# david-wb/tiny-diffusion

Hardware: AMD Instinct MI355X
Metric: train images/s (q_sample+fwd+MSE+bwd+allreduce+Adam), MNIST 28x28 UNet fp32; 1000-step sample latency in `sample` (higher is better)
Workload: dtype f32; 1 GPU; diffusion.py unconditional MNIST 28x28 UNet, fp32, train step, batch 256/GPU (BASELINE.json configs[1]); global_batch=256, per_gpu_batch=256, parallelism=dp1

## Files before the change

include/tdx.h:

```cpp
#ifndef TDX_H
#define TDX_H

#include <stddef.h>
#include <stdint.h>

#ifdef __cplusplus
extern "C" {
#endif

#define TDX_VERSION 400

#define TDX_E_BADARG (-1)
#define TDX_E_SHAPE (-2)
#define TDX_E_WORKSPACE (-3)
#define TDX_E_STATE (-4)

typedef void* tdx_stream_t;

int tdx_version(void);
const char* tdx_error_string(int code);


int tdx_q_sample(const float* x0, const float* noise, const int64_t* t,
                 const float* sqrt_ac, const float* sqrt_1mac, float* x_t,
// ... 65 lines not shown
int tdx_final_conv_backward(const float* in, const float* g_out, const float* w, float* g_in, float* dw, float* db,
                            float* scratch, int B, int H, int W, int cout, tdx_stream_t stream);

int tdx_conv3x3_fwd(const float* in, const float* wpk, const float* bias, float* out,
                    int B, int H, int W, int cin, int cout, int flags,
                    const float* in_scale, const float* in_shift,
                    const float* out_scale, const float* out_shift,
                    float* stats_partial, tdx_stream_t stream);
int tdx_conv3x3_fwd_splitk(const float* in, const float* wpk, const float* bias, float* out,
                           int B, int H, int W, int cin, int cout, int flags,
                           const float* in_scale, const float* in_shift,
                           const float* out_scale, const float* out_shift,
                           float* scratch, size_t scratch_floats, tdx_stream_t stream);
size_t tdx_conv3x3_splitk_scratch_floats(int B, int H, int W, int cin, int cout);
int tdx_conv3x3_wino_ok(int B, int H, int W, int cin, int cout);
int tdx_pack_conv3x3_wino(const float* w_oihw, float* u_fwd, float* u_dgrad, int cout, int cin, tdx_stream_t stream);
int tdx_conv3x3_fwd_wino(const float* in, const float* u, const float* bias, float* out, int B, int H, int W,
                         int cin, int cout, int flags, const float* out_scale, const float* out_shift,
                         float* stats_partial, tdx_stream_t stream);
int tdx_conv3x3_fwd_wino_infer(const float* in, const float* u, const float* bias, float* out, int B, int H, int W,
                               int cin, int cout, const float* out_scale, const float* out_shift, float* scratch,
                               size_t scratch_floats, tdx_stream_t stream);
int tdx_conv3x3_train_algo(int B, int H, int W, int cin, int cout, int role);
int tdx_conv3x3_infer_algo(int B, int H, int W, int cin, int cout);
int tdx_conv3x3_wgrad_wino_splits(int B, int H, int W, int cin, int cout);
int tdx_conv3x3_wgrad_wino(const float* in, const float* dy, float* dw_slabs, int B, int H, int W, int cin, int cout,
                           tdx_stream_t stream);
int tdx_conv3x3_wino_stat_tiles(int B, int H, int W);
int tdx_conv3x3_wino_stat_tile_rows(int B, int H, int W);
int tdx_pack_conv3x3_tiled(const float* w_oihw, float* w_tiled, int cout, int cin, tdx_stream_t stream);
int tdx_conv3x3_fwd_infer(const float* in, const float* w_tiled, const float* bias, float* out, int B, int H, int W,
                          int cin, int cout, const float* out_scale, const float* out_shift, float* scratch,
                          size_t scratch_floats, tdx_stream_t stream);
size_t tdx_conv3x3_infer_scratch_floats(int B, int H, int W, int cin, int cout);
int tdx_conv3x3_fwd_train(const float* in, const float* wpk, const float* bias, float* out, int B, int H, int W,
                          int cin, int cout, int flags, float* stats_partial, float* scratch,
                          size_t scratch_floats, tdx_stream_t stream);
size_t tdx_conv3x3_train_scratch_floats(int B, int H, int W, int cin, int cout);
int tdx_conv3x3_stat_tiles(int B, int H, int W, int cin, int cout);
int tdx_conv3x3_stat_tile_rows(int B, int H, int W, int cin, int cout);
int tdx_conv3x3_shape_ok(int B, int H, int W, int cin, int cout);
int tdx_conv3x3_tile_shape(int B, int H, int W, int cin, int cout, int role);

int tdx_conv3x3_dgrad(const float* dy, const float* w_dgrad, float* dx, int B, int H, int W,
                      int cin, int cout, tdx_stream_t stream);

// ... 184 lines not shown
```

tiny_diffusion_amd/_lib.py:

```python
from __future__ import annotations

import ctypes as C
import os

import torch

from . import _build

_c_float_p = C.c_void_p
_c_i64_p = C.c_void_p
_ptr = C.c_void_p


class TdxError(RuntimeError):
    pass


def _load():
    path = _build.LIB
    if not os.path.exists(path):
        if os.environ.get("TDX_NO_AUTOBUILD"):
            raise TdxError(
                f"{path} not found: build it with `python -m tiny_diffusion_amd._build` "
                "(there is no CPU fallback for the HIP path)"
# ... 29 lines not shown
    "tdx_mse_loss": (C.c_int, [_ptr, _ptr, _ptr, _ptr, C.c_float, C.c_int64, _ptr]),
    "tdx_mse_scratch_bytes": (C.c_size_t, []),
    "tdx_mse_loss_grad": (C.c_int, [_ptr, _ptr, _ptr, _ptr, C.c_float, C.c_int64, _ptr, _ptr]),
    "tdx_adam_step": (C.c_int, [_ptr, _ptr, _ptr, _ptr, C.c_int64, C.c_float, C.c_float, C.c_float,
                                C.c_float, C.c_int, C.c_float, _ptr]),
    "tdx_adam_clip_scratch_bytes": (C.c_size_t, []),
    "tdx_adam_step_clip": (C.c_int, [_ptr, _ptr, _ptr, _ptr, C.c_int64, C.c_float, C.c_float, C.c_float, C.c_float,
                                     C.c_int, C.c_float, C.c_float, _ptr, _ptr, _ptr]),
    "tdx_edge_conv_wgrad_scratch_floats": (C.c_size_t, [C.c_int] * 3),
    "tdx_initial_conv_forward": (C.c_int, [_ptr, _ptr, _ptr, _ptr, C.c_int, C.c_int, C.c_int, C.c_int, C.c_int, _ptr]),
    "tdx_initial_conv_backward": (C.c_int, [_ptr, _ptr, _ptr, _ptr, _ptr, C.c_int, C.c_int, C.c_int, C.c_int, C.c_int,
                                            _ptr]),
    "tdx_final_conv_forward": (C.c_int, [_ptr, _ptr, _ptr, _ptr, C.c_int, C.c_int, C.c_int, C.c_int, _ptr]),
    "tdx_final_conv_backward": (C.c_int, [_ptr, _ptr, _ptr, _ptr, _ptr, _ptr, _ptr, C.c_int, C.c_int, C.c_int, C.c_int,
                                          _ptr]),
    "tdx_pack_conv3x3": (C.c_int, [_ptr, _ptr, _ptr, C.c_int, C.c_int, _ptr]),
    "tdx_conv3x3_wino_ok": (C.c_int, [C.c_int] * 5),
    "tdx_pack_conv3x3_wino": (C.c_int, [_ptr, _ptr, _ptr, C.c_int, C.c_int, _ptr]),
    "tdx_conv3x3_fwd_wino": (C.c_int, [_ptr, _ptr, _ptr, _ptr, C.c_int, C.c_int, C.c_int, C.c_int, C.c_int, C.c_int, _ptr,
                                       _ptr, _ptr, _ptr]),
    "tdx_conv3x3_fwd_wino_infer": (C.c_int, [_ptr, _ptr, _ptr, _ptr, C.c_int, C.c_int, C.c_int, C.c_int, C.c_int, _ptr, _ptr,
                                             _ptr, C.c_size_t, _ptr]),
    "tdx_conv3x3_train_algo": (C.c_int, [C.c_int] * 6),
    "tdx_conv3x3_infer_algo": (C.c_int, [C.c_int] * 5),
    "tdx_conv3x3_wgrad_wino_splits": (C.c_int, [C.c_int] * 5),
    "tdx_conv3x3_wgrad_wino": (C.c_int, [_ptr, _ptr, _ptr, C.c_int, C.c_int, C.c_int, C.c_int, C.c_int, _ptr]),
    "tdx_conv3x3_wino_stat_tiles": (C.c_int, [C.c_int] * 3),
    "tdx_conv3x3_wino_stat_tile_rows": (C.c_int, [C.c_int] * 3),
    "tdx_pack_conv3x3_tiled": (C.c_int, [_ptr, _ptr, C.c_int, C.c_int, _ptr]),
    "tdx_conv3x3_fwd_infer": (C.c_int, [_ptr, _ptr, _ptr, _ptr, C.c_int, C.c_int, C.c_int, C.c_int, C.c_int, _ptr, _ptr,
                                        _ptr, C.c_size_t, _ptr]),
    "tdx_conv3x3_infer_scratch_floats": (C.c_size_t, [C.c_int] * 5),
    "tdx_conv3x3_fwd": (C.c_int, [_ptr, _ptr, _ptr, _ptr, C.c_int, C.c_int, C.c_int, C.c_int, C.c_int,
                                  C.c_int, _ptr, _ptr, _ptr, _ptr, _ptr, _ptr]),
    "tdx_conv3x3_fwd_splitk": (C.c_int, [_ptr, _ptr, _ptr, _ptr, C.c_int, C.c_int, C.c_int, C.c_int, C.c_int,
                                         C.c_int, _ptr, _ptr, _ptr, _ptr, _ptr, C.c_size_t, _ptr]),
    "tdx_conv3x3_splitk_scratch_floats": (C.c_size_t, [C.c_int] * 5),
    "tdx_conv3x3_fwd_train": (C.c_int, [_ptr, _ptr, _ptr, _ptr, C.c_int, C.c_int, C.c_int, C.c_int, C.c_int, C.c_int,
                                        _ptr, _ptr, C.c_size_t, _ptr]),
    "tdx_conv3x3_train_scratch_floats": (C.c_size_t, [C.c_int] * 5),
    "tdx_conv3x3_stat_tiles": (C.c_int, [C.c_int] * 5),
    "tdx_conv3x3_stat_tile_rows": (C.c_int, [C.c_int] * 5),
    "tdx_conv3x3_wgrad_splits": (C.c_int, [C.c_int] * 5),
    "tdx_diag_conv_occupancy": (C.c_int, [C.c_int]),
    "tdx_conv3x3_wgrad_splits_bf16": (C.c_int, [C.c_int] * 5),
    "tdx_conv3x3_fwd_bf16_io": (C.c_int, [_ptr] * 4 + [C.c_int] * 6 + [_ptr] * 5 + [C.c_int, _ptr]),
# ... 133 lines not shown
```

tiny_diffusion_amd/csrc/conv3x3.hip:

```cpp
#include "internal.h"
#include <cstring>
#include <type_traits>

#define BK 32
#define BKP 36

#include "conv_shared.h"

template <int BM, int BN, bool IN_BN, int EPI>
__global__ void __launch_bounds__(256)
conv3x3_igemm_kernel(ConvArgs a) {
  constexpr int WGM = 2, WGN = 2;
  constexpr int WTM = BM / WGM, WTN = BN / WGN;
  constexpr int TM = WTM / 32, TN = WTN / 32;
  constexpr int AI = BM / 32, BI = BN / 32;
  static_assert(TM >= 1 && TN >= 1, "wave tile must hold a 32x32 MFMA tile");

  extern __shared__ __attribute__((aligned(16))) float smem[];
  float* As = smem;
  float* Bs = smem + 2 * BM * BKP;

  const int tid = threadIdx.x;
  const int lane = tid & 63, wave = tid >> 6;
  const int l31 = lane & 31, half = lane >> 5;
// ... 776 lines not shown
  if (!strcmp(key, "time_proj_early")) { g_tdx_time_proj_early = value != 0; return 0; }
  if (!strcmp(key, "time_stage_diag")) { g_tdx_time_stage = value == 6 ? 6 : 14; return 0; }
  if (!strcmp(key, "time_l1_impl")) { g_tdx_time_l1_impl = value; return 0; }
  if (!strcmp(key, "input_copy")) { g_tdx_input_copy = value; return 0; }
  if (!strcmp(key, "conv_dbg")) { g_conv_dbg = value; return 0; }
  if (!strcmp(key, "bf16_materialize")) { g_tdx_bf16_materialize = value ? 1 : 0; return 0; }
  if (!strcmp(key, "bf16_thin")) { g_tdx_bf16_thin = value < 0 ? 0 : value; return 0; }
  if (!strcmp(key, "bf16_ring")) { g_tdx_bf16_ring = value ? 1 : 0; return 0; }
  if (!strcmp(key, "bf16_wgrad9")) { g_tdx_wgrad9 = value ? 1 : 0; return 0; }
  if (!strcmp(key, "bf16_wgrad_swz")) { g_tdx_wgrad_bf16s = value ? 1 : 0; return 0; }
  if (!strcmp(key, "conv_stamp")) { g_conv_stamp = value; g_tdx_probe_stamp = value; return 0; }
  if (!strcmp(key, "wgrad_small")) { g_wgrad_small = value; return 0; }
  if (!strcmp(key, "wino")) { g_tdx_wino = value != 0; return 0; }
  if (!strcmp(key, "wino_infer")) { g_tdx_wino_infer = value != 0; return 0; }
  if (!strcmp(key, "wino_infer_min_units")) { g_tdx_wino_infer_min_units = value >= 0 ? value : 700; return 0; }
  if (!strcmp(key, "wino_infer_ovh")) { g_wino_infer_ovh = value >= 0 ? value : 2; return 0; }
  if (!strcmp(key, "wino_infer_red")) { g_wino_infer_red = value >= 0 ? value : 3; return 0; }
  if (!strcmp(key, "wino_wgrad")) { g_tdx_wino_wgrad = value != 0; return 0; }
  if (!strcmp(key, "wino_wgrad_min_tiles")) { g_tdx_wino_wgrad_min_tiles = value > 0 ? value : 1024; return 0; }
  if (!strcmp(key, "wino_wgrad_target")) { g_tdx_wino_wgrad_target = value > 0 ? value : 512; return 0; }
  if (!strcmp(key, "wino_min_wgs")) { g_tdx_wino_min_wgs = value > 0 ? value : 1; return 0; }
  if (!strcmp(key, "wino_rows")) { g_tdx_wino_rows = value != 0; return 0; }
  if (!strcmp(key, "wino_rows_min_stages")) { g_tdx_wino_rows_min_stages = value > 0 ? value : 16; return 0; }
  if (!strcmp(key, "infer_ring")) { g_tdx_infer_ring = value != 0; return 0; }
  if (!strcmp(key, "infer_stages")) { g_infer_stages = value == 3 ? 3 : 4; return 0; }
  if (!strcmp(key, "infer_splits")) { g_infer_splits = value > 0 ? value : 0; return 0; }
  if (!strcmp(key, "infer_ovh")) { g_infer_ovh = value >= 0 ? value : 4; return 0; }
  if (!strcmp(key, "infer_red")) { g_infer_red = value >= 0 ? value : 12; return 0; }
  if (!strcmp(key, "infer_cus")) { g_tdx_infer_cus = value > 0 && value <= 256 ? value : 256; return 0; }
  if (!strcmp(key, "wgrad9_wgs")) { g_wgrad9_wgs = value > 0 ? value : 0; return 0; }
  if (!strcmp(key, "wgrad_plan")) { g_wgrad_plan = value; return 0; }
  if (!strcmp(key, "wgrad_rounds")) { g_wgrad_rounds = value; return 0; }
  if (!strcmp(key, "conv_dma")) { g_conv_dma = value; return 0; }
  if (!strcmp(key, "wgrad_target")) { g_wgrad_target = value > 0 ? value : 2048; return 0; }
  if (!strcmp(key, "wgrad_target_big")) { g_wgrad_target_big = value > 0 ? value : 0; return 0; }
  return TDX_E_BADARG;
}

static TileCfg pick_tile(int64_t M, int cout) {
  const TileCfg cands[3] = {{128, 128}, {128, 64}, {64, 64}};
  if (g_force_tile >= 1 && g_force_tile <= 3 && cout % cands[g_force_tile - 1].bn == 0)
    return cands[g_force_tile - 1];
  for (int i = 0; i < 3; ++i) {
    if (cout % cands[i].bn) continue;
    if (i == 2) return cands[i];
    const int64_t tiles = ((M + cands[i].bm - 1) / cands[i].bm) * (cout / cands[i].bn);
// ... 1187 lines not shown
```

tiny_diffusion_amd/csrc/conv3x3_wino.hip:

```cpp
#include "internal.h"
#include "conv_shared.h"

extern unsigned* g_tdx_diag_buffer;
extern size_t g_tdx_diag_bytes;
extern int g_tdx_probe_stamp;

constexpr int WT = 64;
constexpr int WN = 64;
constexpr int WK = 8;
constexpr int A_ST = 16 * WT * WK;
constexpr int B_ST = 16 * WN * WK;
constexpr int STAGE = A_ST + B_ST;

struct WinoArgs {
  const float* in;
  const float* u;
  const float* bias;
  float* out;
  const float* out_scale;
  const float* out_shift;
  float* stats;
  int B, H, W, Cin, Cout, th, tw, NT, tilesN, M;
  float rcp_tpi, rcp_tw;
  int per;
  int compact;
  unsigned long long* stamps;
};

constexpr int OLD = 68;
constexpr int TAB_OFF = 2 * STAGE;
typedef unsigned u32x4 __attribute__((ext_vector_type(4)));

template <int EPI, int XH = -1>
__device__ __forceinline__ void wino_epilogue(const WinoArgs& a, float* out, const float* bias, f32x16 (&acc)[16], float* smem,
                                              int tblk, int n0, int wm, int wn, int l31, int half, int tid,
                                              const f32x4* xin = nullptr) {
#if defined(__HIP_DEVICE_COMPILE__)
  const unsigned* tab = reinterpret_cast<const unsigned*>(smem + TAB_OFF);
  const int cl = wn * 32 + l31, col = n0 + cl;
  const float bv = bias ? bias[col] : 0.f;
  float osc = 1.f, osh = 0.f;
  if (EPI == EPI_BNRELU) { osc = a.out_scale[col]; osh = a.out_shift[col]; }
  float csum = 0.f, cnt = 0.f;
  float* ot = smem;
  f32x4 pv[8];
#pragma unroll
  for (int r = 0; r < 16; ++r) {
    if (XH >= 0 && (r & 3) == 0) {
#pragma unroll
      for (int p = 0; p < 8; ++p) pv[p] = xin[(p * 4 + (r >> 2)) * 64];
    }
    auto M = [&](int p) { return XH >= 0 && (p >> 3) != XH ? pv[p & 7][r & 3] : acc[p][r]; };
    float s0[4], s1[4];
#pragma unroll
    for (int nu = 0; nu < 4; ++nu) {
      s0[nu] = M(0 + nu) + M(4 + nu) + M(8 + nu);
      s1[nu] = M(4 + nu) - M(8 + nu) - M(12 + nu);
    }
    float y[4] = {s0[0] + s0[1] + s0[2], s0[1] - s0[2] - s0[3], s1[0] + s1[1] + s1[2], s1[1] - s1[2] - s1[3]};
    const int tl = wm * 32 + (r & 3) + 8 * (r >> 2) + 4 * half;
    const unsigned m = tab[2 * tl + 1];
#pragma unroll
    for (int q = 0; q < 4; ++q) {
      float val = y[q] + bv;
      if (EPI == EPI_BNRELU) val = fmaxf(fmaf(val, osc, osh), 0.f);
      const bool ok = (m >> q) & 1u;
      if (XH < 0) ot[(tl * 4 + q) * OLD + cl] = val;
      csum += ok ? val : 0.f;
      cnt += ok ? 1.f : 0.f;
      y[q] = ok ? val : 0.f;
    }
    acc[0][r] = y[0]; acc[1][r] = y[1]; acc[4][r] = y[2]; acc[5][r] = y[3];
    acc[2][r] = (m & 1u) ? 1.f : 0.f;
    acc[3][r] = (m & 2u) ? 1.f : 0.f;
    acc[6][r] = (m & 4u) ? 1.f : 0.f;
    acc[7][r] = (m & 8u) ? 1.f : 0.f;
  }
  if (XH >= 0) {
    __syncthreads();
#pragma unroll
    for (int r = 0; r < 16; ++r) {
      const int tl = wm * 32 + (r & 3) + 8 * (r >> 2) + 4 * half;
      ot[(tl * 4 + 0) * OLD + cl] = acc[0][r]; ot[(tl * 4 + 1) * OLD + cl] = acc[1][r];
      ot[(tl * 4 + 2) * OLD + cl] = acc[4][r]; ot[(tl * 4 + 3) * OLD + cl] = acc[5][r];
    }
  }
  __syncthreads();
  {
    const auto rsrc_out = __builtin_amdgcn_make_buffer_rsrc(out, 0, (int)((int64_t)a.M * a.Cout * 4), 0x00020000);
    const int c4 = (tid & 15) * 4, q = (tid >> 4) & 3;
    const unsigned qoff = (unsigned)((((q >> 1) * a.W + (q & 1)) * a.Cout + n0 + c4) * 4);
    const uint2* tab2 = reinterpret_cast<const uint2*>(tab);
    const float* src = ot + (tid >> 4) * OLD + c4;
#pragma unroll
    for (int i = 0; i < 16; ++i) {
      const uint2 e = tab2[4 * i + (tid >> 6)];
      const unsigned off = ((e.y >> q) & 1u) ? e.x + qoff : 0x80000000u;
      const f32x4 v = *reinterpret_cast<const f32x4*>(src + i * 16 * OLD);
      __builtin_amdgcn_raw_buffer_store_b128(__builtin_bit_cast(u32x4, v), rsrc_out, off, 0, 0);
    }
  }
  if (EPI == EPI_STATS) {
    float* red = smem + 256 * OLD;
    const float s = csum + __shfl_xor(csum, 32, 64);
    const float n = cnt + __shfl_xor(cnt, 32, 64);
    if (half == 0) { red[wm * 64 + cl] = s; red[128 + wm * 64 + cl] = n; }
    __syncthreads();
    if (tid < 64) {
      const float ts = red[tid] + red[64 + tid];
      const float tn = red[128 + tid] + red[192 + tid];
      red[256 + tid] = tn > 0.f ? ts / tn : 0.f;
      a.stats[((size_t)tblk * 2 + 0) * a.Cout + n0 + tid] = ts;
    }
    __syncthreads();
    const float mean = red[256 + cl];
    float q = 0.f;
#pragma unroll
    for (int r = 0; r < 16; ++r) {
      const float d0 = acc[0][r] - mean, d1 = acc[1][r] - mean, d2 = acc[4][r] - mean, d3 = acc[5][r] - mean;
      q = fmaf(d0 * acc[2][r], d0, q); q = fmaf(d1 * acc[3][r], d1, q);
      q = fmaf(d2 * acc[6][r], d2, q); q = fmaf(d3 * acc[7][r], d3, q);
    }
    q += __shfl_xor(q, 32, 64);
    __syncthreads();
    if (half == 0) red[wm * 64 + cl] = q;
    __syncthreads();
    if (tid < 64) a.stats[((size_t)tblk * 2 + 1) * a.Cout + n0 + tid] = red[tid] + red[64 + tid];
  }
#endif
}

#if defined(__HIP_DEVICE_COMPILE__)
__device__ __forceinline__ float s_add(float x, float y) { float r; asm("v_add_f32 %0, %1, %2" : "=v"(r) : "v"(x), "v"(y)); return r; }
__device__ __forceinline__ float s_sub(float x, float y) { float r; asm("v_sub_f32 %0, %1, %2" : "=v"(r) : "v"(x), "v"(y)); return r; }
__device__ __forceinline__ f32x4 add4(f32x4 x, f32x4 y) { return f32x4{s_add(x[0], y[0]), s_add(x[1], y[1]), s_add(x[2], y[2]), s_add(x[3], y[3])}; }
__device__ __forceinline__ f32x4 sub4(f32x4 x, f32x4 y) { return f32x4{s_sub(x[0], y[0]), s_sub(x[1], y[1]), s_sub(x[2], y[2]), s_sub(x[3], y[3])}; }
#endif

__device__ __forceinline__ int div_rcp(int n, int d, float r, int* rem) {
  int q = (int)((float)n * r);
  int m = n - q * d;
  if (m < 0) { --q; m += d; }
  else if (m >= d) { ++q; m -= d; }
  *rem = m;
  return q;
}

template <int EPI, bool SPLITK, bool ROWS>
__global__ void __launch_bounds__(256)
conv3x3_wino_kernel(WinoArgs a) {
// ... 274 lines not shown
        }
      };
      if (PEEL) stage(std::true_type{}, 0);
      for (int s = PEEL ? 1 : 0; s < ns; ++s) stage(std::false_type{}, s);
      asm volatile("s_waitcnt vmcnt(0) lgkmcnt(0)\n\ts_barrier" ::: "memory");
    }
    if (a.stamps) { t_loop = __builtin_amdgcn_s_memrealtime(); c_loop = __builtin_amdgcn_s_memtime() - c_loop; }
    if (SPLITK)
      wino_epilogue<EPI_PLAIN>(a, a.out + (size_t)blockIdx.y * (size_t)a.M * a.Cout, nullptr, acc, smem, tblk, n0, wm, wn, l31, half, tid);
    else
      wino_epilogue<EPI>(a, a.out, a.bias, acc, smem, tblk, n0, wm, wn, l31, half, tid);
  }
  if (a.stamps && tid == 0) {
    asm volatile("s_waitcnt vmcnt(0)" ::: "memory");
    unsigned long long* o = a.stamps + 8 * ((size_t)blockIdx.y * gridDim.x + blockIdx.x);
    o[0] = t_entry; o[1] = t_issued; o[2] = t_landed; o[3] = t_loop; o[4] = __builtin_amdgcn_s_memrealtime();
    o[5] = c_loop;
    o[6] = __builtin_amdgcn_s_getreg(4 | (0 << 6) | (31 << 11));
    o[7] = __builtin_amdgcn_s_getreg(20 | (0 << 6) | (3 << 11)) & 0xf;
  }
#endif
}

__global__ void __launch_bounds__(512) pack_wino_batch_kernel(TdxWinoPackBatch b) {
  int u = 0;
  while (u + 1 < b.count && (int)blockIdx.x >= b.start[u + 1]) ++u;
  const int cin = b.cin[u], cout = b.cout[u], cin_real = b.cin_real[u];
  const int blk = blockIdx.x - b.start[u];
  const int nkb = cin / 8;
  const int cb = blk / nkb, kb = blk - cb * nkb;
  const int cl = threadIdx.x >> 3, k8 = threadIdx.x & 7;
  const int co = cb * 64 + cl, ci = kb * 8 + k8;
  float g[9];
#pragma unroll
  for (int tap = 0; tap < 9; ++tap) g[tap] = ci < cin_real ? b.w[u][((size_t)co * cin_real + ci) * 9 + tap] : 0.f;
  float gg[4][3], U[16];
#pragma unroll
  for (int c = 0; c < 3; ++c) {
    gg[0][c] = g[c];
    gg[1][c] = 0.5f * (g[c] + g[3 + c] + g[6 + c]);
    gg[2][c] = 0.5f * (g[c] - g[3 + c] + g[6 + c]);
    gg[3][c] = g[6 + c];
  }
#pragma unroll
  for (int r = 0; r < 4; ++r) {
    U[r * 4 + 0] = gg[r][0];
// ... 53 lines not shown
  pack_wino_batch_kernel<<<blocks, 512, 0, to_stream(stream)>>>(*b);
  TDX_CHECK_LAUNCH();
  return 0;
}

int tdx_pack_conv3x3_wino_pad(const float* w_oihw, float* u_fwd, float* u_dgrad, int cout, int cin_real, int cin,
                              tdx_stream_t stream) {
  if (!w_oihw || cout <= 0 || cin <= 0 || cin_real <= 0 || cin_real > cin) return TDX_E_BADARG;
  if (cin % 64 || cout % 64) return TDX_E_SHAPE;
  if (!u_fwd && !u_dgrad) return 0;
  TdxWinoPackBatch b{};
  b.count = 1;
  b.w[0] = w_oihw; b.uf[0] = u_fwd; b.ud[0] = u_dgrad; b.cout[0] = cout; b.cin[0] = cin; b.cin_real[0] = cin_real;
  return tdx_pack_conv3x3_wino_batch(&b, stream);
}

extern "C" int tdx_pack_conv3x3_wino(const float* w_oihw, float* u_fwd, float* u_dgrad, int cout, int cin,
                                     tdx_stream_t stream) {
  return tdx_pack_conv3x3_wino_pad(w_oihw, u_fwd, u_dgrad, cout, cin, cin, stream);
}

int g_tdx_wino_rows = 1;
int g_tdx_wino_rows_min_stages = 16;

int tdx_conv3x3_wino_launch(const float* in, const float* u, const float* bias, float* out, int B, int H, int W,
                            int cin, int cout, int flags, const float* out_scale, const float* out_shift,
                            float* stats_partial, int splits, int per, tdx_stream_t stream) {
  if (!in || !u || !out) return TDX_E_BADARG;
  if (!tdx_conv3x3_wino_ok(B, H, W, cin, cout)) return TDX_E_SHAPE;
  if (flags & ~(TDX_CONV_OUT_BNRELU | TDX_CONV_OUT_STATS)) return TDX_E_BADARG;
  if ((flags & TDX_CONV_OUT_BNRELU) && (!out_scale || !out_shift)) return TDX_E_BADARG;
  if ((flags & TDX_CONV_OUT_STATS) && (!stats_partial || (flags & TDX_CONV_OUT_BNRELU))) return TDX_E_BADARG;
  if (splits < 1 || (splits > 1 && (per < 1 || (int64_t)per * (splits - 1) >= cin / WK))) return TDX_E_BADARG;
  WinoArgs a{};
  a.in = in; a.u = u; a.bias = bias; a.out = out; a.out_scale = out_scale; a.out_shift = out_shift;
  a.stats = stats_partial;
  a.B = B; a.H = H; a.W = W; a.Cin = cin; a.Cout = cout;
  a.th = (H + 1) / 2; a.tw = (W + 1) / 2;
  a.NT = B * a.th * a.tw;
  a.rcp_tpi = 1.0f / (float)(a.th * a.tw); a.rcp_tw = 1.0f / (float)a.tw;
  a.tilesN = cout / WN;
  a.M = B * H * W;
  a.per = per;
  a.compact = cdiv(a.NT, WT) < 64;
  const dim3 grid(a.compact ? cdiv(a.NT, WT) * a.tilesN : (cdiv(a.NT, WT) + 7) / 8 * 8 * a.tilesN, splits);
  a.stamps = g_tdx_probe_stamp == 3 && g_tdx_diag_buffer && (size_t)grid.x * grid.y * 64 <= g_tdx_diag_bytes
                 ? reinterpret_cast<unsigned long long*>(g_tdx_diag_buffer) : nullptr;
  const size_t lds = (size_t)2 * STAGE * sizeof(float) + WT * 2 * sizeof(unsigned);
  hipStream_t st = to_stream(stream);
#define TDX_WINO_LAUNCH(EPI_, SPL_, ROWS_)                                                                       \
  do {                                                                                                           \
    auto kern = conv3x3_wino_kernel<EPI_, SPL_, ROWS_>;                                                          \
    static bool attr_set = false;                                                                                \
    if (!attr_set) {                                                                                             \
      hipError_t e = hipFuncSetAttribute(reinterpret_cast<const void*>(kern),                                    \
                                         hipFuncAttributeMaxDynamicSharedMemorySize, (int)lds);                  \
      if (e != hipSuccess) return (int)e;                                                                        \
      attr_set = true;                                                                                           \
    }                                                                                                            \
    kern<<<grid, 256, lds, st>>>(a);                                                                             \
  } while (0)
  const bool rows = g_tdx_wino_rows && cin / WK >= g_tdx_wino_rows_min_stages;
  if (splits > 1) TDX_WINO_LAUNCH(EPI_PLAIN, true, false);
  else if (flags & TDX_CONV_OUT_BNRELU) TDX_WINO_LAUNCH(EPI_BNRELU, false, false);
  else if (flags & TDX_CONV_OUT_STATS) {
    if (rows) TDX_WINO_LAUNCH(EPI_STATS, false, true);
    else TDX_WINO_LAUNCH(EPI_STATS, false, false);
  } else if (rows) TDX_WINO_LAUNCH(EPI_PLAIN, false, true);
  else TDX_WINO_LAUNCH(EPI_PLAIN, false, false);
#undef TDX_WINO_LAUNCH
  TDX_CHECK_LAUNCH();
  return 0;
}

extern "C" int tdx_conv3x3_fwd_wino(const float* in, const float* u, const float* bias, float* out, int B, int H, int W,
                                    int cin, int cout, int flags, const float* out_scale, const float* out_shift,
                                    float* stats_partial, tdx_stream_t stream) {
  return tdx_conv3x3_wino_launch(in, u, bias, out, B, H, W, cin, cout, flags, out_scale, out_shift, stats_partial, 1, 0,
                                 stream);
}

constexpr int GT8 = 8;
constexpr int XS_F = GT8 * 16 * 64;
constexpr int ES_F = GT8 * 4 * 64;
constexpr int WST_F = XS_F + ES_F;
constexpr int WNST = 3;
constexpr int WG_MAX_CHUNK = 1024;
constexpr int WG_XCH_F = 4 * 8 * 16 * 64;
constexpr size_t WG_LDS = 131072;
static_assert((size_t)WNST * WST_F * 4 + (size_t)WG_MAX_CHUNK * 4 <= WG_LDS && (size_t)WG_XCH_F * 4 <= WG_LDS, "LDS");

struct WinoWgArgs {
  const float* in;
// ... 330 lines not shown
```

tiny_diffusion_amd/csrc/internal.h:

```cpp
#pragma once
#include "common.h"

int tdx_copy_floats(const float* src, float* dst, size_t n, hipStream_t st);
int tdx_copy_segments(const float* const* src, float* const* dst, const size_t* n, int count, hipStream_t st);
int tdx_pixel_sum(const void* g, float* out, int B, int HW, int C, hipStream_t st, int io16 = 0);
int tdx_reduce_partials(const float* partial, float* out, int nblk, int stride, int count,
                        hipStream_t st);
int tdx_initial_conv_fwd(const float* x, const float* w, const float* bias, void* out, int B, int H,
                         int W, int cin, int cout_real, hipStream_t st, int io16 = 0);
int tdx_small_conv_wgrad_blocks(int B, int H, int W);
int tdx_small_conv_partial_width(void);
int tdx_initial_conv_wgrad(const float* x, const void* g, float* partial, float* dw, float* db,
                           int B, int H, int W, int cin, int cout_real, hipStream_t st, int io16 = 0);
int tdx_initial_conv_dgrad(const void* g_x0, const float* w, float* g_x, int B, int H, int W, int cin,
                           int cout_real, hipStream_t st, int io16 = 0);
int tdx_final_conv_fwd(const void* in, const float* w, const float* bias, float* out, int B, int H,
                       int W, int cout, hipStream_t st, int io16 = 0);
int tdx_final_conv_fwd_psample(const void* in, const float* w, const float* bias, float* eps_out, int B, int H, int W,
                               int cout, float* x, const float* z, const float* coef, const int32_t* t_idx,
                               uint64_t seed, int philox, int64_t* counter_dec, hipStream_t st, int io16 = 0,
                               int64_t elem0 = 0, const int64_t* tau = nullptr);
int tdx_final_conv_dgrad(const float* g_out, const float* w, void* g_in, int B, int H, int W,
                         int cout, hipStream_t st, int io16 = 0);
int tdx_final_conv_wgrad(const void* in, const float* g_out, float* partial, float* dw, float* db,
// ... 23 lines not shown
#define TDX_PACK_MAX 13
struct TdxPackBatch {
  const float* w[TDX_PACK_MAX];
  float* wf[TDX_PACK_MAX];
  float* wd[TDX_PACK_MAX];
  int cout[TDX_PACK_MAX], cin[TDX_PACK_MAX], cin_real[TDX_PACK_MAX], chunk_start[TDX_PACK_MAX];
  int count;
};
int tdx_pack_conv3x3_batch(TdxPackBatch* b, tdx_stream_t stream);
struct TdxWinoPackBatch {
  const float* w[TDX_PACK_MAX];
  float* uf[TDX_PACK_MAX];
  float* ud[TDX_PACK_MAX];
  int cout[TDX_PACK_MAX], cin[TDX_PACK_MAX], cin_real[TDX_PACK_MAX], start[TDX_PACK_MAX];
  int count;
};
int tdx_pack_conv3x3_wino_batch(TdxWinoPackBatch* b, tdx_stream_t stream);
extern "C" int tdx_conv3x3_wino_ok(int B, int H, int W, int cin, int cout);
extern "C" int tdx_conv3x3_wino_stat_tiles(int B, int H, int W);
extern "C" int tdx_conv3x3_wino_stat_tile_rows(int B, int H, int W);
extern int g_tdx_wino, g_tdx_wino_min_wgs;
extern int g_tdx_wino_wgrad, g_tdx_wino_wgrad_min_tiles, g_tdx_wino_wgrad_target;
extern int g_tdx_wino_rows, g_tdx_wino_rows_min_stages;
extern "C" int tdx_conv3x3_wgrad_wino_splits(int B, int H, int W, int cin, int cout);
extern "C" int tdx_conv3x3_wgrad_wino(const float* in, const float* dy, float* dw_slabs, int B, int H, int W, int cin, int cout,
                                      tdx_stream_t stream);
extern int g_tdx_wino_infer_min_units;
extern int g_tdx_wino_infer;
int tdx_conv3x3_wino_launch(const float* in, const float* u, const float* bias, float* out, int B, int H, int W,
                            int cin, int cout, int flags, const float* out_scale, const float* out_shift,
                            float* stats_partial, int splits, int per, tdx_stream_t stream);
int tdx_conv3x3_fwd_wino_infer_ex(const float* in, const float* u, const float* bias, float* out, int B, int H, int W,
                                  int cin, int cout, const float* out_scale, const float* out_shift, float* scratch,
                                  size_t scratch_floats, tdx_stream_t stream, TdxSplitDefer* defer, TdxPoolFuse* pool);
int tdx_pack_conv3x3_tiled_batch(TdxPackBatch* b, tdx_stream_t stream);
int tdx_pack_conv3x3_tiled_pad(const float* w_oihw, float* w_tiled, int cout, int cin_real, int cin, tdx_stream_t stream);
int tdx_pack_conv3x3_batch_bf16(TdxPackBatch* b, tdx_stream_t stream);
int tdx_pack_conv3x3_pad(const float* w_oihw, float* w_fwd, float* w_dgrad, int cout, int cin_real,
                         int cin, tdx_stream_t stream);
int tdx_conv3x3_wgrad_reduce_pad(const float* dw_slabs, float* dw_oihw, int splits, int cout, int cin,
                                 int cin_real, tdx_stream_t stream);
int tdx_time_embed_bwd_ex(const float* tf, const int64_t* y, const float* const* P, float* const* G,
                          const float* pre, const float* emb, const float* const* gk, const int* ldg,
                          const int* widths, float* scratch, int B, int ncls, hipStream_t st,
                          const int64_t* t_i64 = nullptr, int td = 0, int parts = 7);
int tdx_bn_moments(const float* stats_partial, int tiles, int tile_rows, int64_t count, int C, double* mom,
// ... 77 lines not shown
```

Measured before the change: 27090 images/s.

## Split Winograd conv tail wave into half-width workgroups to balance CUs

```diff
diff --git a/include/tdx.h b/include/tdx.h
--- a/include/tdx.h
+++ b/include/tdx.h
@@ -111,6 +111,9 @@
                                int cin, int cout, const float* out_scale, const float* out_shift, float* scratch,
                                size_t scratch_floats, tdx_stream_t stream);
 int tdx_conv3x3_train_algo(int B, int H, int W, int cin, int cout, int role);
+int tdx_conv3x3_wino_tail_plan(int B, int H, int W, int cout, int cus, int* plan);
+int tdx_conv3x3_wino_tail_wg(int B, int H, int W, int cout, int cus, int id, int* wg);
+int tdx_conv3x3_wino_tail_last(int* plan);
 int tdx_conv3x3_infer_algo(int B, int H, int W, int cin, int cout);
 int tdx_conv3x3_wgrad_wino_splits(int B, int H, int W, int cin, int cout);
 int tdx_conv3x3_wgrad_wino(const float* in, const float* dy, float* dw_slabs, int B, int H, int W, int cin, int cout,
diff --git a/tiny_diffusion_amd/_lib.py b/tiny_diffusion_amd/_lib.py
--- a/tiny_diffusion_amd/_lib.py
+++ b/tiny_diffusion_amd/_lib.py
@@ -75,6 +75,9 @@
     "tdx_conv3x3_fwd_wino_infer": (C.c_int, [_ptr, _ptr, _ptr, _ptr, C.c_int, C.c_int, C.c_int, C.c_int, C.c_int, _ptr, _ptr,
                                              _ptr, C.c_size_t, _ptr]),
     "tdx_conv3x3_train_algo": (C.c_int, [C.c_int] * 6),
+    "tdx_conv3x3_wino_tail_plan": (C.c_int, [C.c_int] * 5 + [C.POINTER(C.c_int)]),
+    "tdx_conv3x3_wino_tail_wg": (C.c_int, [C.c_int] * 6 + [C.POINTER(C.c_int)]),
+    "tdx_conv3x3_wino_tail_last": (C.c_int, [C.POINTER(C.c_int)]),
     "tdx_conv3x3_infer_algo": (C.c_int, [C.c_int] * 5),
     "tdx_conv3x3_wgrad_wino_splits": (C.c_int, [C.c_int] * 5),
     "tdx_conv3x3_wgrad_wino": (C.c_int, [_ptr, _ptr, _ptr, C.c_int, C.c_int, C.c_int, C.c_int, C.c_int, _ptr]),
diff --git a/tiny_diffusion_amd/csrc/conv3x3.hip b/tiny_diffusion_amd/csrc/conv3x3.hip
--- a/tiny_diffusion_amd/csrc/conv3x3.hip
+++ b/tiny_diffusion_amd/csrc/conv3x3.hip
@@ -822,6 +822,8 @@
   if (!strcmp(key, "wino_min_wgs")) { g_tdx_wino_min_wgs = value > 0 ? value : 1; return 0; }
   if (!strcmp(key, "wino_rows")) { g_tdx_wino_rows = value != 0; return 0; }
   if (!strcmp(key, "wino_rows_min_stages")) { g_tdx_wino_rows_min_stages = value > 0 ? value : 16; return 0; }
+  if (!strcmp(key, "wino_tail_max_rounds")) { g_tdx_wino_tail_max_rounds = value >= 0 ? value : 3; return 0; }
+  if (!strcmp(key, "wino_tail")) { g_tdx_wino_tail = value & 3; return 0; }
   if (!strcmp(key, "infer_ring")) { g_tdx_infer_ring = value != 0; return 0; }
   if (!strcmp(key, "infer_stages")) { g_infer_stages = value == 3 ? 3 : 4; return 0; }
   if (!strcmp(key, "infer_splits")) { g_infer_splits = value > 0 ? value : 0; return 0; }
diff --git a/tiny_diffusion_amd/csrc/conv3x3_wino.hip b/tiny_diffusion_amd/csrc/conv3x3_wino.hip
--- a/tiny_diffusion_amd/csrc/conv3x3_wino.hip
+++ b/tiny_diffusion_amd/csrc/conv3x3_wino.hip
@@ -1,3 +1,4 @@
+#include <mutex>
 #include "internal.h"
 #include "conv_shared.h"
 
@@ -25,17 +26,40 @@
   int per;
   int compact;
   unsigned long long* stamps;
+  int nb;
+  int half_f0;
 };
+
+__host__ __device__ inline void wino_real_wg(int f, int nb, int tilesN, int compact, int* tblk, int* nblk) {
+  if (compact) { *tblk = f / tilesN; *nblk = f - *tblk * tilesN; return; }
+  const int g8 = 8 * tilesN, nfull = (nb >> 3) * g8;
+  if (f < nfull) {
+    const int xb = f / g8, xr = f - xb * g8;
+    *tblk = xb * 8 + (xr & 7); *nblk = xr >> 3;
+  } else {
+    const int rem = nb & 7, fr = f - nfull;
+    *nblk = fr / rem; *tblk = (nb & ~7) + (fr - *nblk * rem);
+  }
+}
+static int wino_real_id(int f, int nb, int tilesN, int compact) {
+  if (compact) return f;
+  int tblk, nblk;
+  wino_real_wg(f, nb, tilesN, compact, &tblk, &nblk);
+  return (tblk >> 3) * 8 * tilesN + nblk * 8 + (tblk & 7);
+}
 
 constexpr int OLD = 68;
 constexpr int TAB_OFF = 2 * STAGE;
 typedef unsigned u32x4 __attribute__((ext_vector_type(4)));
 
-template <int EPI, int XH = -1>
+template <int EPI, int XH = -1, bool HALF = false>
 __device__ __forceinline__ void wino_epilogue(const WinoArgs& a, float* out, const float* bias, f32x16 (&acc)[16], float* smem,
                                               int tblk, int n0, int wm, int wn, int l31, int half, int tid,
                                               const f32x4* xin = nullptr) {
 #if defined(__HIP_DEVICE_COMPILE__)
+  static_assert(!HALF || XH >= 0, "the half-width workgroup runs the row split");
+  constexpr bool ACTIVE = !HALF || XH == 0;
+  constexpr int NW = HALF ? 32 : 64;
   const unsigned* tab = reinterpret_cast<const unsigned*>(smem + TAB_OFF);
   const int cl = wn * 32 + l31, col = n0 + cl;
   const float bv = bias ? bias[col] : 0.f;
@@ -45,7 +69,7 @@
   float* ot = smem;
   f32x4 pv[8];
 #pragma unroll
-  for (int r = 0; r < 16; ++r) {
+  for (int r = 0; r < (ACTIVE ? 16 : 0); ++r) {
     if (XH >= 0 && (r & 3) == 0) {
 #pragma unroll
       for (int p = 0; p < 8; ++p) pv[p] = xin[(p * 4 + (r >> 2)) * 64];
@@ -79,7 +103,7 @@
   if (XH >= 0) {
     __syncthreads();
 #pragma unroll
-    for (int r = 0; r < 16; ++r) {
+    for (int r = 0; r < (ACTIVE ? 16 : 0); ++r) {
       const int tl = wm * 32 + (r & 3) + 8 * (r >> 2) + 4 * half;
       ot[(tl * 4 + 0) * OLD + cl] = acc[0][r]; ot[(tl * 4 + 1) * OLD + cl] = acc[1][r];
       ot[(tl * 4 + 2) * OLD + cl] = acc[4][r]; ot[(tl * 4 + 3) * OLD + cl] = acc[5][r];
@@ -88,15 +112,16 @@
   __syncthreads();
   {
     const auto rsrc_out = __builtin_amdgcn_make_buffer_rsrc(out, 0, (int)((int64_t)a.M * a.Cout * 4), 0x00020000);
-    const int c4 = (tid & 15) * 4, q = (tid >> 4) & 3;
+    constexpr int LP = NW / 4, RI = 256 / LP;
+    const int c4 = (tid & (LP - 1)) * 4, q = (tid / LP) & 3;
     const unsigned qoff = (unsigned)((((q >> 1) * a.W + (q & 1)) * a.Cout + n0 + c4) * 4);
     const uint2* tab2 = reinterpret_cast<const uint2*>(tab);
-    const float* src = ot + (tid >> 4) * OLD + c4;
-#pragma unroll
-    for (int i = 0; i < 16; ++i) {
-      const uint2 e = tab2[4 * i + (tid >> 6)];
+    const float* src = ot + (tid / LP) * OLD + c4;
+#pragma unroll
+    for (int i = 0; i < LP; ++i) {
+      const uint2 e = tab2[(RI / 4) * i + tid / (4 * LP)];
       const unsigned off = ((e.y >> q) & 1u) ? e.x + qoff : 0x80000000u;
-      const f32x4 v = *reinterpret_cast<const f32x4*>(src + i * 16 * OLD);
+      const f32x4 v = *reinterpret_cast<const f32x4*>(src + i * RI * OLD);
       __builtin_amdgcn_raw_buffer_store_b128(__builtin_bit_cast(u32x4, v), rsrc_out, off, 0, 0);
     }
   }
@@ -104,9 +129,9 @@
     float* red = smem + 256 * OLD;
     const float s = csum + __shfl_xor(csum, 32, 64);
     const float n = cnt + __shfl_xor(cnt, 32, 64);
-    if (half == 0) { red[wm * 64 + cl] = s; red[128 + wm * 64 + cl] = n; }
+    if (ACTIVE && half == 0) { red[wm * 64 + cl] = s; red[128 + wm * 64 + cl] = n; }
     __syncthreads();
-    if (tid < 64) {
+    if (tid < NW) {
       const float ts = red[tid] + red[64 + tid];
       const float tn = red[128 + tid] + red[192 + tid];
       red[256 + tid] = tn > 0.f ? ts / tn : 0.f;
@@ -116,16 +141,16 @@
     const float mean = red[256 + cl];
     float q = 0.f;
 #pragma unroll
-    for (int r = 0; r < 16; ++r) {
+    for (int r = 0; r < (ACTIVE ? 16 : 0); ++r) {
       const float d0 = acc[0][r] - mean, d1 = acc[1][r] - mean, d2 = acc[4][r] - mean, d3 = acc[5][r] - mean;
       q = fmaf(d0 * acc[2][r], d0, q); q = fmaf(d1 * acc[3][r], d1, q);
       q = fmaf(d2 * acc[6][r], d2, q); q = fmaf(d3 * acc[7][r], d3, q);
     }
     q += __shfl_xor(q, 32, 64);
     __syncthreads();
-    if (half == 0) red[wm * 64 + cl] = q;
+    if (ACTIVE && half == 0) red[wm * 64 + cl] = q;
     __syncthreads();
-    if (tid < 64) a.stats[((size_t)tblk * 2 + 1) * a.Cout + n0 + tid] = red[tid] + red[64 + tid];
+    if (tid < NW) a.stats[((size_t)tblk * 2 + 1) * a.Cout + n0 + tid] = red[tid] + red[64 + tid];
   }
 #endif
 }
@@ -446,6 +471,193 @@
 #endif
 }
 
+template <int EPI>
+__global__ void __launch_bounds__(256)
+conv3x3_wino_half_kernel(WinoArgs a) {
+#if defined(__HIP_DEVICE_COMPILE__)
+  static_assert(EPI != EPI_BNRELU, "training launches only");
+  typedef __attribute__((address_space(3))) void* lds_ptr_t;
+  extern __shared__ __attribute__((aligned(16))) float smem[];
+  const unsigned long long t_entry = a.stamps ? __builtin_amdgcn_s_memrealtime() : 0ull;
+  const int tid = threadIdx.x;
+  const int lane = tid & 63;
+  const int wave = __builtin_amdgcn_readfirstlane(tid >> 6);
+  const int l31 = lane & 31, half = lane >> 5;
+  const int wm = wave & 1, wh = wave >> 1;
+  int tblk, nblk;
+  wino_real_wg(a.half_f0 + ((int)blockIdx.x >> 1), a.nb, a.tilesN, a.compact, &tblk, &nblk);
+  const int T0 = tblk * WT;
+  if (T0 >= a.NT) return;
+  const int n0 = nblk * WN + ((int)blockIdx.x & 1) * 32;
+  const int tpi = a.th * a.tw;
+
+  if (tid < WT) {
+    const int T = T0 + tid;
+    const bool tv = T < a.NT;
+    int rem, tx;
+    const int b = div_rcp(T, tpi, a.rcp_tpi, &rem);
+    const int ty = div_rcp(rem, a.tw, a.rcp_tw, &tx);
+    const bool r1 = 2 * ty + 1 < a.H, c1 = 2 * tx + 1 < a.W;
+    unsigned* tab = reinterpret_cast<unsigned*>(smem + TAB_OFF);
+    tab[2 * tid] = tv ? (unsigned)(((b * a.H + 2 * ty) * a.W + 2 * tx) * a.Cout * 4) : 0u;
+    tab[2 * tid + 1] = tv ? (1u | (c1 ? 2u : 0u) | (r1 ? 4u : 0u) | (r1 && c1 ? 8u : 0u)) : 0u;
+  }
+  const auto rsrc_in = __builtin_amdgcn_make_buffer_rsrc(const_cast<float*>(a.in), 0, (int)((int64_t)a.M * a.Cin * 4), 0x00020000);
+  const auto rsrc_u = __builtin_amdgcn_make_buffer_rsrc(const_cast<float*>(a.u), 0, a.Cout * 16 * a.Cin * 4, 0x00020000);
+  constexpr unsigned OOB = 0x80000000u;
+  unsigned a_off[4][2];
+#pragma unroll
+  for (int g = 0; g < 2; ++g) {
+    const int T = T0 + g * 32 + (lane >> 1);
+    const bool tv = T < a.NT;
+    int rem, tx;
+    const int b = div_rcp(T, tpi, a.rcp_tpi, &rem);
+    const int ty = div_rcp(rem, a.tw, a.rcp_tw, &tx);
+#pragma unroll
+    for (int j = 0; j < 4; ++j) {
+      const int px = 4 * wave + j;
+      const int ih = 2 * ty - 1 + (px >> 2), iw = 2 * tx - 1 + (px & 3);
+      const bool ok = tv && (unsigned)ih < (unsigned)a.H && (unsigned)iw < (unsigned)a.W;
+      a_off[j][g] = ok ? (unsigned)((((b * a.H + ih) * a.W + iw) * a.Cin + (lane & 1) * 4) * 4) : OOB;
+    }
+  }
+  const unsigned u_base = (unsigned)(nblk * (a.Cin / WK)) * (unsigned)(B_ST * 4) +
+                          (unsigned)(wave * 4 * 2048 + ((int)blockIdx.x & 1) * 1024 + lane * 16);
+  const int ns = a.Cin / WK;
+  auto piece = [&](int i, int buf, int k) {
+    const int sc = k < ns ? k : ns - 1;
+    float* Ab = smem + buf * STAGE;
+    float* Bb = Ab + A_ST;
+    if (i < 4)
+      __builtin_amdgcn_raw_ptr_buffer_load_lds(rsrc_u, (lds_ptr_t)(Bb + (wave * 4 + i) * 256), 16, u_base + i * 2048,
+                                               (unsigned)sc * (unsigned)(B_ST * 4), 0, 0);
+    else
+      __builtin_amdgcn_raw_ptr_buffer_load_lds(rsrc_in, (lds_ptr_t)(Ab + (4 * wave + ((i - 4) >> 1)) * 512 + ((i - 4) & 1) * 256), 16,
+                                               a_off[(i - 4) >> 1][(i - 4) & 1], (unsigned)(sc * WK * 4), 0, 0);
+  };
+  f32x16 acc[16];
+  const f32x16 zero16 = {0.f, 0.f, 0.f, 0.f, 0.f, 0.f, 0.f, 0.f, 0.f, 0.f, 0.f, 0.f, 0.f, 0.f, 0.f, 0.f};
+#pragma unroll
+  for (int i = 0; i < 12; ++i) piece(i, 0, 0);
+#pragma unroll
+  for (int i = 0; i < 12; ++i) piece(i, 1, 1);
+  unsigned long long t_issued = 0, t_landed = 0, t_loop = 0, c_loop = 0;
+  if (a.stamps) t_issued = __builtin_amdgcn_s_memrealtime();
+  asm volatile("s_waitcnt vmcnt(12) lgkmcnt(0)\n\ts_barrier" ::: "memory");
+  if (a.stamps) { t_landed = __builtin_amdgcn_s_memrealtime(); c_loop = __builtin_amdgcn_s_memtime(); }
+  auto body = [&](auto Hc) {
+    constexpr int H = decltype(Hc)::value;
+    f32x4 d[12], v[8], t[4], bq[5], nbq[2];
+    const int lofs = wm * 256 + l31 * 8 + half * 4;
+    const int bofs = A_ST + 8 * H * 256 + l31 * 8 + half * 4;
+    auto trow = [&](int x, int c) {
+      if (H == 0) t[c] = x == 0 ? sub4(d[c], d[8 + c]) : add4(d[4 + c], d[8 + c]);
+      else t[c] = x == 0 ? sub4(d[4 + c], d[c]) : sub4(d[c], d[8 + c]);
+    };
+    auto vcol = [&](int x, int c) {
+      f32x4& o = v[4 * x + c];
+      if (c == 0) o = sub4(t[0], t[2]);
+      else if (c == 1) o = add4(t[1], t[2]);
+      else if (c == 2) o = sub4(t[2], t[1]);
+      else o = sub4(t[1], t[3]);
+    };
+    constexpr int RA = 0, RB = H == 0 ? 2 : 1, RC = H == 0 ? 1 : 2;
+    {
+      const float* Ab = smem + 4 * H * 512 + lofs;
+      const float* Bb = smem + bofs;
+#pragma unroll
+      for (int c = 0; c < 4; ++c) {
+        d[4 * RA + c] = *reinterpret_cast<const f32x4*>(Ab + (4 * RA + c) * 512);
+        d[4 * RB + c] = *reinterpret_cast<const f32x4*>(Ab + (4 * RB + c) * 512);
+      }
+      nbq[0] = *reinterpret_cast<const f32x4*>(Bb);
+      nbq[1] = *reinterpret_cast<const f32x4*>(Bb + 256);
+#pragma unroll
+      for (int c = 0; c < 4; ++c) d[4 * RC + c] = *reinterpret_cast<const f32x4*>(Ab + (4 * RC + c) * 512);
+#pragma unroll
+      for (int c = 0; c < 4; ++c) trow(0, c);
+#pragma unroll
+      for (int c = 0; c < 4; ++c) vcol(0, c);
+    }
+    auto stage = [&](auto first_c, int s) {
+      constexpr bool FIRST = decltype(first_c)::value;
+      const int cb = s & 1;
+      const float* Bb = smem + cb * STAGE + bofs;
+      const float* An = smem + (cb ^ 1) * STAGE + 4 * H * 512 + lofs;
+      const float* Bn = smem + (cb ^ 1) * STAGE + bofs;
+      bq[0] = nbq[0]; bq[1] = nbq[1];
+      __builtin_amdgcn_sched_barrier(0);
+#pragma unroll
+      for (int g = 0; g < 8; ++g) {
+        const int cur = g % 5;
+        if (FIRST) acc[g] = __builtin_amdgcn_mfma_f32_32x32x2f32(v[g][0], bq[cur][0], zero16, 0, 0, 0);
+        else acc[g] = __builtin_amdgcn_mfma_f32_32x32x2f32(v[g][0], bq[cur][0], acc[g], 0, 0, 0);
+        if (g == 2) bq[1] = *reinterpret_cast<const f32x4*>(Bb + 6 * 256);
+        if (g == 3) bq[2] = *reinterpret_cast<const f32x4*>(Bb + 7 * 256);
+        if (g == 4) {
+          asm volatile("s_waitcnt vmcnt(0) lgkmcnt(0)\n\ts_barrier" ::: "memory");
+#pragma unroll
+          for (int c = 0; c < 4; ++c) {
+            d[4 * RA + c] = *reinterpret_cast<const f32x4*>(An + (4 * RA + c) * 512);
+            d[4 * RB + c] = *reinterpret_cast<const f32x4*>(An + (4 * RB + c) * 512);
+          }
+        }
+        if (g == 5) {
+#pragma unroll
+          for (int c = 0; c < 4; ++c) d[4 * RC + c] = *reinterpret_cast<const f32x4*>(An + (4 * RC + c) * 512);
+        }
+        if (g == 6) {
+#pragma unroll
+          for (int c = 0; c < 4; ++c) trow(0, c);
+        }
+        if (g == 7) { vcol(0, 2); vcol(0, 3); }
+        __builtin_amdgcn_sched_barrier(0);
+        acc[g] = __builtin_amdgcn_mfma_f32_32x32x2f32(v[g][1], bq[cur][1], acc[g], 0, 0, 0);
+        if (g < 2) { trow(1, 2 * g); trow(1, 2 * g + 1); }
+        else if (g < 4) { vcol(1, 2 * g - 4); vcol(1, 2 * g - 3); }
+        else piece(g - 4, cb, s + 2);
+        __builtin_amdgcn_sched_barrier(0);
+        acc[g] = __builtin_amdgcn_mfma_f32_32x32x2f32(v[g][2], bq[cur][2], acc[g], 0, 0, 0);
+        if (g < 4) bq[(g + 2) % 5] = *reinterpret_cast<const f32x4*>(Bb + (g + 2) * 256);
+        if (g == 4) { nbq[0] = *reinterpret_cast<const f32x4*>(Bn); nbq[1] = *reinterpret_cast<const f32x4*>(Bn + 256); }
+        if (g == 6) { vcol(0, 0); vcol(0, 1); }
+        __builtin_amdgcn_sched_barrier(0);
+        acc[g] = __builtin_amdgcn_mfma_f32_32x32x2f32(v[g][3], bq[cur][3], acc[g], 0, 0, 0);
+        if (g >= 4) { piece(4 + 2 * (g - 4), cb, s + 2); piece(5 + 2 * (g - 4), cb, s + 2); }
+        __builtin_amdgcn_sched_barrier(0);
+      }
+    };
+    stage(std::true_type{}, 0);
+    for (int s = 1; s < ns; ++s) stage(std::false_type{}, s);
+    asm volatile("s_waitcnt vmcnt(0) lgkmcnt(0)\n\ts_barrier" ::: "memory");
+    if (a.stamps) { t_loop = __builtin_amdgcn_s_memrealtime(); c_loop = __builtin_amdgcn_s_memtime() - c_loop; }
+    if (H == 1) {
+      f32x4* xo = reinterpret_cast<f32x4*>(smem) + wm * 2048 + lane;
+#pragma unroll
+      for (int pp = 0; pp < 8; ++pp)
+#pragma unroll
+        for (int r4 = 0; r4 < 4; ++r4) {
+          const f32x16& x = acc[pp];
+          xo[(pp * 4 + r4) * 64] = f32x4{x[4 * r4], x[4 * r4 + 1], x[4 * r4 + 2], x[4 * r4 + 3]};
+        }
+    }
+    __syncthreads();
+    wino_epilogue<EPI, H, true>(a, a.out, a.bias, acc, smem, tblk, n0, wm, 0, l31, half, tid,
+                                reinterpret_cast<const f32x4*>(smem) + wm * 2048 + lane);
+  };
+  if (wh) body(std::integral_constant<int, 1>{});
+  else body(std::integral_constant<int, 0>{});
+  if (a.stamps && tid == 0) {
+    asm volatile("s_waitcnt vmcnt(0)" ::: "memory");
+    unsigned long long* o = a.stamps + 8 * (size_t)blockIdx.x;
+    o[0] = t_entry; o[1] = t_issued; o[2] = t_landed; o[3] = t_loop; o[4] = __builtin_amdgcn_s_memrealtime();
+    o[5] = c_loop;
+    o[6] = __builtin_amdgcn_s_getreg(4 | (0 << 6) | (31 << 11));
+    o[7] = (__builtin_amdgcn_s_getreg(20 | (0 << 6) | (3 << 11)) & 0xf) | 16u;
+  }
+#endif
+}
+
 __global__ void __launch_bounds__(512) pack_wino_batch_kernel(TdxWinoPackBatch b) {
   int u = 0;
   while (u + 1 < b.count && (int)blockIdx.x >= b.start[u + 1]) ++u;
@@ -545,6 +757,68 @@
 
 int g_tdx_wino_rows = 1;
 int g_tdx_wino_rows_min_stages = 16;
+
+int g_tdx_wino_tail = 1;
+int g_tdx_wino_tail_max_rounds = 3;
+
+struct WinoTailPlan { int full_grid, full_real, half_wgs; };
+static WinoTailPlan wino_tail_plan(int nb, int tilesN, int cus, bool tail) {
+  const int compact = nb < 64, F = nb * tilesN;
+  WinoTailPlan p{compact ? F : (nb + 7) / 8 * 8 * tilesN, F, 0};
+  const int r = cus > 0 ? F % cus : 0;
+  if (!tail || r == 0 || 2 * r > cus) return p;
+  p.full_real = F - r;
+  p.full_grid = p.full_real ? wino_real_id(p.full_real - 1, nb, tilesN, compact) + 1 : 0;
+  p.half_wgs = 2 * r;
+  return p;
+}
+
+static int wino_device_cus() {
+  static std::once_flag once;
+  static int cus = 0;
+  std::call_once(once, [] {
+    int dev = 0, n = 0;
+    if (hipGetDevice(&dev) == hipSuccess && hipDeviceGetAttribute(&n, hipDeviceAttributeMultiprocessorCount, dev) == hipSuccess)
+      cus = n;
+  });
+  return cus;
+}
+
+static WinoTailPlan g_wino_last_plan;
+
+extern "C" int tdx_conv3x3_wino_tail_plan(int B, int H, int W, int cout, int cus, int* plan) {
+  if (!plan || B <= 0 || H <= 0 || W <= 0 || cout <= 0 || cout % WN || cus <= 0) return TDX_E_BADARG;
+  const int nb = tdx_conv3x3_wino_stat_tiles(B, H, W);
+  const WinoTailPlan p = wino_tail_plan(nb, cout / WN, cus, true);
+  plan[0] = p.full_grid; plan[1] = p.full_real; plan[2] = p.half_wgs; plan[3] = nb;
+  return 0;
+}
+
+extern "C" int tdx_conv3x3_wino_tail_wg(int B, int H, int W, int cout, int cus, int id, int* wg) {
+  int plan[4];
+  if (!wg || id < 0 || tdx_conv3x3_wino_tail_plan(B, H, W, cout, cus, plan)) return TDX_E_BADARG;
+  const int nb = plan[3], tilesN = cout / WN, compact = nb < 64;
+  int tblk, nblk;
+  if (id < plan[0]) {
+    const int xb = id / (8 * tilesN), xr = id % (8 * tilesN);
+    tblk = compact ? id / tilesN : xb * 8 + (xr & 7);
+    nblk = compact ? id - tblk * tilesN : xr >> 3;
+    if (tblk >= nb) return 0;
+    wg[0] = tblk; wg[1] = 2 * nblk;
+    return 2;
+  }
+  const int j = id - plan[0];
+  if (j >= plan[2]) return TDX_E_BADARG;
+  wino_real_wg(plan[1] + (j >> 1), nb, tilesN, compact, &tblk, &nblk);
+  wg[0] = tblk; wg[1] = 2 * nblk + (j & 1);
+  return 1;
+}
+
+extern "C" int tdx_conv3x3_wino_tail_last(int* plan) {
+  if (!plan) return TDX_E_BADARG;
+  plan[0] = g_wino_last_plan.full_grid; plan[1] = g_wino_last_plan.full_real; plan[2] = g_wino_last_plan.half_wgs;
+  return 0;
+}
 
 int tdx_conv3x3_wino_launch(const float* in, const float* u, const float* bias, float* out, int B, int H, int W,
                             int cin, int cout, int flags, const float* out_scale, const float* out_shift,
@@ -565,33 +839,52 @@
   a.tilesN = cout / WN;
   a.M = B * H * W;
   a.per = per;
-  a.compact = cdiv(a.NT, WT) < 64;
-  const dim3 grid(a.compact ? cdiv(a.NT, WT) * a.tilesN : (cdiv(a.NT, WT) + 7) / 8 * 8 * a.tilesN, splits);
-  a.stamps = g_tdx_probe_stamp == 3 && g_tdx_diag_buffer && (size_t)grid.x * grid.y * 64 <= g_tdx_diag_bytes
+  a.nb = cdiv(a.NT, WT);
+  a.compact = a.nb < 64;
+  const bool train = splits == 1 && !(flags & TDX_CONV_OUT_BNRELU);
+  const int role_bit = (flags & TDX_CONV_OUT_STATS) ? 1 : 2;
+  const int cus = wino_device_cus();
+  const WinoTailPlan plan = wino_tail_plan(a.nb, a.tilesN, cus, train && (g_tdx_wino_tail & role_bit) && cus > 0 &&
+                                                                    a.nb * a.tilesN / cus <= g_tdx_wino_tail_max_rounds);
+  if (train) g_wino_last_plan = plan;
+  const dim3 grid(plan.full_grid, splits);
+  a.stamps = g_tdx_probe_stamp == 3 && g_tdx_diag_buffer &&
+                     ((size_t)grid.x * grid.y + plan.half_wgs) * 64 <= g_tdx_diag_bytes
                  ? reinterpret_cast<unsigned long long*>(g_tdx_diag_buffer) : nullptr;
   const size_t lds = (size_t)2 * STAGE * sizeof(float) + WT * 2 * sizeof(unsigned);
   hipStream_t st = to_stream(stream);
-#define TDX_WINO_LAUNCH(EPI_, SPL_, ROWS_)                                                                       \
+#define TDX_WINO_LAUNCH_(KERN_, GRID_)                                                                           \
   do {                                                                                                           \
-    auto kern = conv3x3_wino_kernel<EPI_, SPL_, ROWS_>;                                                          \
-    static bool attr_set = false;                                                                                \
-    if (!attr_set) {                                                                                             \
-      hipError_t e = hipFuncSetAttribute(reinterpret_cast<const void*>(kern),                                    \
-                                         hipFuncAttributeMaxDynamicSharedMemorySize, (int)lds);                  \
-      if (e != hipSuccess) return (int)e;                                                                        \
-      attr_set = true;                                                                                           \
-    }                                                                                                            \
-    kern<<<grid, 256, lds, st>>>(a);                                                                             \
+    auto kern = KERN_;                                                                                           \
+    static std::once_flag once;                                                                                  \
+    static hipError_t attr_e = hipSuccess;                                                                       \
+    std::call_once(once, [&] {                                                                                   \
+      attr_e = hipFuncSetAttribute(reinterpret_cast<const void*>(kern),                                          \
+                                   hipFuncAttributeMaxDynamicSharedMemorySize, (int)lds);                        \
+    });                                                                                                          \
+    if (attr_e != hipSuccess) return (int)attr_e;                                                                \
+    kern<<<GRID_, 256, lds, st>>>(a);                                                                            \
   } while (0)
+#define TDX_WINO_LAUNCH(EPI_, SPL_, ROWS_) TDX_WINO_LAUNCH_((conv3x3_wino_kernel<EPI_, SPL_, ROWS_>), grid)
   const bool rows = g_tdx_wino_rows && cin / WK >= g_tdx_wino_rows_min_stages;
-  if (splits > 1) TDX_WINO_LAUNCH(EPI_PLAIN, true, false);
+  if (grid.x == 0) {}
+  else if (splits > 1) TDX_WINO_LAUNCH(EPI_PLAIN, true, false);
   else if (flags & TDX_CONV_OUT_BNRELU) TDX_WINO_LAUNCH(EPI_BNRELU, false, false);
   else if (flags & TDX_CONV_OUT_STATS) {
     if (rows) TDX_WINO_LAUNCH(EPI_STATS, false, true);
     else TDX_WINO_LAUNCH(EPI_STATS, false, false);
   } else if (rows) TDX_WINO_LAUNCH(EPI_PLAIN, false, true);
   else TDX_WINO_LAUNCH(EPI_PLAIN, false, false);
+  if (plan.half_wgs) {
+    TDX_CHECK_LAUNCH();
+    a.half_f0 = plan.full_real;
+    if (a.stamps) a.stamps += 8 * (size_t)grid.x;
+    const dim3 hgrid(plan.half_wgs);
+    if (flags & TDX_CONV_OUT_STATS) TDX_WINO_LAUNCH_(conv3x3_wino_half_kernel<EPI_STATS>, hgrid);
+    else TDX_WINO_LAUNCH_(conv3x3_wino_half_kernel<EPI_PLAIN>, hgrid);
+  }
 #undef TDX_WINO_LAUNCH
+#undef TDX_WINO_LAUNCH_
   TDX_CHECK_LAUNCH();
   return 0;
 }
diff --git a/tiny_diffusion_amd/csrc/internal.h b/tiny_diffusion_amd/csrc/internal.h
--- a/tiny_diffusion_amd/csrc/internal.h
+++ b/tiny_diffusion_amd/csrc/internal.h
@@ -69,6 +69,7 @@
 extern int g_tdx_wino, g_tdx_wino_min_wgs;
 extern int g_tdx_wino_wgrad, g_tdx_wino_wgrad_min_tiles, g_tdx_wino_wgrad_target;
 extern int g_tdx_wino_rows, g_tdx_wino_rows_min_stages;
+extern int g_tdx_wino_tail, g_tdx_wino_tail_max_rounds;
 extern "C" int tdx_conv3x3_wgrad_wino_splits(int B, int H, int W, int cin, int cout);
 extern "C" int tdx_conv3x3_wgrad_wino(const float* in, const float* dy, float* dw_slabs, int B, int H, int W, int cin, int cout,
                                       tdx_stream_t stream);
```

After: 27200 images/s, median of 6. No clear change (+0.4%).
